# rohitgirdhar/AttentionalPoolingAction

Measured on AMD Instinct MI355X. Metric: images/sec attn-pool fwd+bwd, Nx14x14x2048, 393 classes, higher is better.
Workload: dtype f32; 1 GPU; cfg002 attentional-pooling head fwd + softmax-xent + bwd, per-GPU batch 32 x 14x14x2048 f32 features, K=393, M=1 (class-agnostic bottom-up map), dropout keep=0.2; X/dX rotated over 4 buffer sets (411 MB live); global_batch=32, parallelism=dp1, softmax_att=False, hip_graph=False, allreduce=none

## Files before the change

### attentionalpoolingaction_amd/csrc/apa_capi.hip

```cpp
#include <stdarg.h>
#include <stdio.h>

#include "../../include/apa_pose_cache.h"
#include "apa_internal.h"
#include "../../include/apa_clip_epoch.h"

namespace apa {

static thread_local char g_err[512] = "no error";

void set_error(const char* fmt, ...) {
  va_list ap;
  va_start(ap, fmt);
  vsnprintf(g_err, sizeof(g_err), fmt, ap);
  va_end(ap);
}

int hip_fail(hipError_t e, const char* what) {
  set_error("HIP error %d (%s) at %s", (int)e, hipGetErrorString(e), what);
  return APA_ERR_HIP;
}

__global__ void zero_words_kernel(uint32_t* __restrict__ p, size_t n) {
  const size_t stride = (size_t)gridDim.x * blockDim.x;
// ... 396 lines not shown
  if (d.ws_bytes < need) {
    set_error("%s: workspace too small (%zu < %zu = apa_attn_pool_rank_workspace_bytes)", fn, d.ws_bytes, need);
    return APA_ERR_WORKSPACE;
  }
  return APA_OK;
}

extern "C" size_t apa_attn_pool_rank_workspace_bytes(int N, int P, int C, int Ca, int K, int extra) {
  if (N <= 0 || P <= 0 || C <= 0 || Ca <= 0 || K <= 0 || extra < 1 || extra > APA_RANK_MAX - 1) return 0;
  return m1r_workspace_bytes(N, P, C, Ca, K, extra + 1);
}

static int rank_fwd_run(const PoolCall& d, const RankCall& rk, const M1Fwd& f) {
  M1Call c;
  const int rc = m1_call_fill(c, d, &f, nullptr);
  return rc != APA_OK ? rc : m1r_forward(c, rk, f);
}
static int rank_bwd_run(const PoolCall& d, const RankCall& rk, const M1Bwd& b) {
  M1Call c;
  const int rc = m1_call_fill(c, d, nullptr, &b);
  return rc != APA_OK ? rc : m1r_backward(c, rk, b);
}

extern "C" int apa_attn_pool_rank_fwd(const apa_rank_maps* rank, const void* X, const void* Xatt, const float* Wa,
                                      const float* ba, const float* Wt, const float* bt, float* logits, float* att,
                                      float* zsave, float* abar, void* ws, size_t ws_bytes, int N, int P, int C, int Ca,
                                      int K, int M, unsigned flags, float keep_prob, uint64_t seed, uint64_t offset,
                                      int dtype, void* stream) {
  const PoolCall d = pool_call({N, P, C, Ca, K, M, dtype}, flags, keep_prob, seed, offset, ws, ws_bytes, stream);
  const M1Fwd f{X, Xatt, Wa, ba, Wt, bt, logits, att, zsave, abar};
  RankCall rk = {};
  const int rc = rank_check("apa_attn_pool_rank_fwd", rank, d, &f, nullptr, &rk);
  return rc != APA_OK ? rc : rank_fwd_run(d, rk, f);
}

// ... 1143 lines not shown
```

### attentionalpoolingaction_amd/csrc/apa_internal.h

```cpp
#pragma once
#include <hip/hip_runtime.h>
#include <hip/hip_ext.h>
#include <stddef.h>
#include <stdint.h>
#include <stdlib.h>
#include <type_traits>

#include "../../include/apa.h"
#include "apa_colsum.h"
#include "apa_gather.h"

namespace apa {

void set_error(const char* fmt, ...);
int hip_fail(hipError_t e, const char* what);
int zero_fill(void* p, size_t bytes, hipStream_t st);

constexpr int APA_MAX_DEVICES = 64;
inline int current_device_slot() {
  int d = 0;
  if (hipGetDevice(&d) != hipSuccess || d < 0) d = 0;
  return d % APA_MAX_DEVICES;
}
template <typename T> struct PerDevice {
// ... 130 lines not shown
bool gemm_bf16_eligible(const GemmDesc& d);
int gemm_bf16_launch(const GemmDesc& d, int splits, int k_per_split, hipStream_t st);
bool gemm_bf16_twin_ok(const GemmDesc& d, int splits, int k_per_split);
bool gemm_bf16_zp_serves(const GemmDesc& d);
bool gemm_bf16_wide_serves(int M, int N, int K);
int gemm_bf16_wide_tile_rows(int M, int N, int K);
int gemm_bf16_mid_dropout(const void* A, long lda, const void* B, long ldb, void* C, long ldc, int M, int N,
                          int K, float inv_keep, const uint8_t* maskbits, hipStream_t st);

constexpr unsigned APA_PUBLIC_FLAGS = 0x3FFu;
constexpr unsigned APA_IFLAG_ATT_READY = 1u << 24;
constexpr unsigned APA_IFLAG_NO_ATT_WGRAD = 1u << 25;
constexpr unsigned APA_IFLAG_NO_DX = 1u << 26;
constexpr unsigned APA_IFLAG_FINALIZE_LAUNCH = 1u << 27;
constexpr unsigned APA_IFLAG_FOLD_TILE16 = 1u << 28;

struct M1Xent {
  const int64_t* labels = nullptr;
  float* loss = nullptr;
  float* G = nullptr;
  float gscale = 0.f, lscale = 0.f;
  bool done = false;
  bool deferred = false;
  float* logits = nullptr;
  float* probs = nullptr;
  int64_t* pred = nullptr;
  int kind = 0;
  const float* mlabels = nullptr;
  float pos_weight = 1.f;
  bool finished = false;
// ... 41 lines not shown
  int pool_bwd, bwd_w, bwd_pix;
  int fused, keep_bits, relu_input;
  int S, ppb, nblk, cw;
  int logits, logits_nv4, logits_nsub;
  int head, head_ug, head_mv;
  int gemv, reduce, rng_bump, cat_fwd, cat_bwd;
};
extern thread_local M1Trace* g_m1_trace;
inline M1Trace* m1_trace() { return g_m1_trace; }
struct M1FwdRoute {
  int folded;
  int launches;
};
extern thread_local unsigned g_m1_iflags;
extern thread_local M1FwdRoute g_m1_fwd_route;

enum M1Act { M1_ACT_ID = 0, M1_ACT_RELU = 1, M1_ACT_SOFTMAX = 2 };
struct M1Fwd {
  const void *X, *Xatt; const float *Wa, *ba, *Wt, *bt; float *logits, *att, *zsave, *abar; void* topdown = nullptr;
};
struct M1Bwd {
  const void *X, *Xatt; const float *Wa, *Wt, *bt, *att, *zsave, *abar, *G; void *dX, *dXatt; float *dWa, *dba, *dWt, *dbt;
};
struct M1Call {
  int N, P, C, Ca, K, dtype; unsigned flags; hipStream_t st; const CatFeat* cat;
  int act, pool_act;
  bool fused, train, rank1, ext, relu_input, no_dx, small, gemv2;
  M1Pool pool; M1Plan pl;
  float *pacc, *pstat, *pdwa, *pdba, *dz, *dzatt, *gemm_ws, *cat_e;
  float* sn;
  uint8_t* maskbits;
  const uint8_t* maskbits_in;
  RngKeyArgs key; float inv_keep; uint64_t* bump;
  const float* ex; float exs;
  hipEvent_t ev0, ev1, td_ready, grad_ready;
  bool gather; int T; M1Gather ga;
};
inline int64_t* m1_gathered_labels(void* ws, const M1Plan& pl) {
  return reinterpret_cast<int64_t*>(static_cast<char*>(ws) + pl.off_pdwa);
}
int m1_call_fill(M1Call& c, const PoolCall& d, const M1Fwd* f, const M1Bwd* b, const M1Xent* xf = nullptr);
int m1_forward(const M1Call& c, const M1Fwd& io, M1Xent* xf = nullptr);
int m1_backward(const M1Call& c, const M1Bwd& io, const M1Xent* xf = nullptr);
bool m1_supported(int C, int Ca, int dtype, bool fused);
bool m1_no_dx_supported(int C, int dtype, bool train);
template <typename F> inline int m1_fused_train(bool fused, bool train, F&& go) {
  if (fused) return train ? go(std::true_type{}, std::true_type{}) : go(std::true_type{}, std::false_type{});
  return train ? go(std::false_type{}, std::true_type{}) : go(std::false_type{}, std::false_type{});
}
template <typename Fn> inline int m1_pool_form(const M1Call& c, Fn&& go) {
  if (c.gather) return m1_fused_train(c.fused, c.train, [&](auto F, auto TR) { return go(F, TR, std::true_type{}); });
  return m1_fused_train(c.fused, c.train, [&](auto F, auto TR) { return go(F, TR, std::false_type{}); });
// ... 35 lines not shown
int m1r_forward(const M1Call& c, const RankCall& rk, const M1Fwd& io);
int m1r_backward(const M1Call& c, const RankCall& rk, const M1Bwd& io);
bool m1_cat_supported(int J);
int m1_cat_forward(const M1Call& c, const M1Fwd& io);
int m1_cat_backward(const M1Call& c, const M1Bwd& io);

bool m1_small_supported(int C, int K);
inline bool m1_small_route_ok(int C, int K, const float* G, const float* Wt, const float* zsave, bool any_ck = false) {
  return (any_ck || m1_small_supported(C, K)) && (((uintptr_t)G | (uintptr_t)Wt | (uintptr_t)zsave) & 15) == 0;
}
int m1_bwd_small(const float* G, const float* Wt, const float* zsave, const float* abar,
                 const float* bt, float* dz, float* dWt, float* dbt, float* sn, int N, int C, int K,
                 hipStream_t st);
bool m1_logits2_supported(int C, int K);
size_t m1_logits2_ws_bytes(int N, int C, int K);
struct M1Fold { const float* pacc; const float* pstat; int S, P; };
bool m1_logits2_fold_supported(int N, int C, int S);
int m1_logits2(float* z, const float* Wt, float* abar, const float* bt, float* logits,
               float* part_ws, int N, int C, int K, hipStream_t st, const M1Fold* fold = nullptr);
int m1_logits2_partials(float* z, const float* Wt, float* part_ws, int N, int C, int K, hipStream_t st,
                        const M1Fold* fold, int* nparts);
bool m1_logits_ml_supported(int N, int C, int K);
int m1_logits2_ml(float* z, const float* Wt, float* abar, const float* bt, const M1Xent& xf, float* logits,
                  float* part_ws, int N, int C, int K, hipStream_t st, const M1Fold* fold);
int ml_loss_rows(int kind, const float* labels, float pos_weight, const float* logits, float* loss, float* G, int N,
                 int K, float wt, float grad_scale, hipStream_t st);
int clip_loss_finish(const float* x, const float* dws, float* loss, float* dw, float* db, int B, int rows, int K,
                     float lscale, hipStream_t st);
int clip_scores_launch(const char* fn, int kind, const float* logits, const float* w, const float* b,
                       const int64_t* labels, float* pooled, float* tatt, float* scores, int64_t* pred, float* loss,
                       int B, int F, int K, hipStream_t st);
bool m1_bwd_head_supported(int N, int C, int K);
// ... 157 lines not shown
```

### attentionalpoolingaction_amd/csrc/apa_m1.hip

```cpp
#include <math.h>

#include "apa_device.h"
#include "apa_internal.h"

namespace apa {

__global__ __launch_bounds__(256) void m1_finalize_fwd_kernel(
    const float* __restrict__ pacc, const float* __restrict__ pstat, int P, int S, int C, int online_softmax, int cw,
    float* __restrict__ z, float* __restrict__ abar, float* __restrict__ att) {
  __shared__ float s_w[256];
  __shared__ float s_red[8];
  const int n = blockIdx.x;
  const int lane = threadIdx.x & 63, wave = threadIdx.x >> 6;
  const float invP = 1.0f / (float)P;
  const float* st = pstat + (size_t)n * S * 4;
  constexpr int FB = 16;
  const bool chan = (int)threadIdx.x < cw;
  const int v = chan ? blockIdx.y * cw + threadIdx.x : 0;
  const float* pa = pacc + (size_t)n * S * C + (v * 4 < C ? v * 4 : 0);
  float4 first[FB];
  if (chan) {
#pragma unroll
    for (int u = 0; u < FB; ++u)
      first[u] = *reinterpret_cast<const float4*>(pa + (size_t)min(u, S - 1) * C);
  }
  float m_s = -INFINITY, l_s = 0.f, a_s = 0.f;
  if ((int)threadIdx.x < S) {
    m_s = st[threadIdx.x * 4];
    l_s = st[threadIdx.x * 4 + 1];
    a_s = st[threadIdx.x * 4 + 2];
  }
  float M = 0.f, invL = 1.f, asum = 0.f;
  if (online_softmax) {
    float mw = wave_max(m_s);
    if (lane == 0) s_red[wave] = mw;
    __syncthreads();
    M = fmaxf(fmaxf(s_red[0], s_red[1]), fmaxf(s_red[2], s_red[3]));
    const float e = ((int)threadIdx.x < S) ? expf(m_s - M) : 0.f;
    float lw = wave_sum(l_s * e);
// ... 1 lines not shown
    __syncthreads();
    invL = 1.0f / ((s_red[4] + s_red[5]) + (s_red[6] + s_red[7]));
    s_w[threadIdx.x] = e * invL * invP;
  } else {
    float aw = wave_sum(a_s);
    if (lane == 0) s_red[wave] = aw;
    s_w[threadIdx.x] = invP;
    __syncthreads();
    asum = (s_red[0] + s_red[1]) + (s_red[2] + s_red[3]);
  }
  __syncthreads();
  if (chan && v * 4 < C) {
    float4 r = make_float4(0.f, 0.f, 0.f, 0.f);
#pragma unroll
    for (int u = 0; u < FB; ++u) {
      if (u < S) {
        const float w = s_w[u];
        r.x = fmaf(first[u].x, w, r.x); r.y = fmaf(first[u].y, w, r.y);
        r.z = fmaf(first[u].z, w, r.z); r.w = fmaf(first[u].w, w, r.w);
      }
    }
    for (int s0 = FB; s0 < S; s0 += FB) {
      float4 a[FB];
#pragma unroll
      for (int u = 0; u < FB; ++u)
        a[u] = *reinterpret_cast<const float4*>(pa + (size_t)min(s0 + u, S - 1) * C);
#pragma unroll
      for (int u = 0; u < FB; ++u) {
        const float w = s0 + u < S ? s_w[s0 + u] : 0.f;
        r.x = fmaf(a[u].x, w, r.x); r.y = fmaf(a[u].y, w, r.y);
        r.z = fmaf(a[u].z, w, r.z); r.w = fmaf(a[u].w, w, r.w);
      }
    }
    *reinterpret_cast<float4*>(z + (size_t)n * C + v * 4) = r;
  }
  if (blockIdx.y == 0) {
    if (online_softmax) {
      float tot = 0.f;
      for (int p = threadIdx.x; p < P; p += 256) {
        const float a = expf(att[(size_t)n * P + p] - M) * invL;
        att[(size_t)n * P + p] = a;
        tot += a;
      }
      tot = wave_sum(tot);
// ... 156 lines not shown
        dwa[e] = fmaf(g[u], x[e], dwa[e]);
      }
      if (STORE && active && p0 + u < p_end) st16(dXa + (size_t)(p0 + u) * Ca + v * EPV, Vec<T>::pack(o));
    }
  }
  if (active) {
#pragma unroll
    for (int e = 0; e < EPV; ++e) pdwa[(size_t)blockIdx.x * Ca + v * EPV + e] = dwa[e];
  }
  if (threadIdx.x == 0) pdba[blockIdx.x] = dba;
}

thread_local M1Trace* g_m1_trace = nullptr;
thread_local unsigned g_m1_iflags = 0;
thread_local M1FwdRoute g_m1_fwd_route = {0, 0};

bool m1_supported(int C, int Ca, int dtype, bool fused) {
  if (dtype == APA_DTYPE_FP8_E4M3) return fused && m1f_supported(C);
  const int epv = dtype == APA_DTYPE_BF16 ? 8 : 4;
  if (!fused && (Ca % epv != 0)) return false;
  return m1s_supported(C, dtype) || m1v_supported(C, dtype) || m1g_supported(C, dtype);
}

M1Plan m1_plan(int N, int P, int C, int Ca, int K) {
  M1Plan pl;
  int S = (512 + N / 2) / N;
  if (S < 1) S = 1;
  int maxS = P >= 8 ? P / 4 : 1;
  if (maxS > 256) maxS = 256;
  if (S > maxS) S = maxS;
// ... 40 lines not shown
  c.train = (flags & APA_FLAG_TRAIN) && keep_prob < 1.0f;
  c.act = (flags & APA_FLAG_SOFTMAX_ATT) ? M1_ACT_SOFTMAX
          : (flags & APA_FLAG_RELU_ATT) ? M1_ACT_RELU : M1_ACT_ID;
  c.pool_act = c.fused ? c.act : M1_ACT_ID;
  c.rank1 = b && (flags & APA_FLAG_DXATT_RANK1) != 0 && !c.fused;
  c.ext = c.train && rng_external(flags);
  c.relu_input = (flags & APA_FLAG_RELU_INPUT) != 0;
  c.no_dx = b && (flags & (APA_IFLAG_NO_DX | APA_FLAG_FROZEN_INPUT)) != 0;
  c.small = b && m1_small_route_ok(C, K, b->G, b->Wt, b->zsave);
  const int epv = dtype == APA_DTYPE_F32 ? 4 : 8;
  c.gemv2 = Ca % epv == 0 && Ca / epv <= 256;
  c.pool = dtype == APA_DTYPE_FP8_E4M3 ? M1_POOL_FP8
           : !c.ext && m1s_supported(C, dtype) ? M1_POOL_STREAM
           : !c.ext && m1v_supported(C, dtype) ? M1_POOL_VEC : M1_POOL_GENERIC;
  c.pl = m1_plan(N, P, C, Ca, K);
  char* w = static_cast<char*>(ws);
  c.pacc = reinterpret_cast<float*>(w + c.pl.off_pacc);
  c.pstat = reinterpret_cast<float*>(w + c.pl.off_pstat);
  c.pdwa = reinterpret_cast<float*>(w + c.pl.off_pdwa);
  c.pdba = reinterpret_cast<float*>(w + c.pl.off_pdba);
  c.sn = c.small ? c.pdba + c.pl.nblk : nullptr;
  c.dz = reinterpret_cast<float*>(w + c.pl.off_dz);
  c.dzatt = c.rank1 ? static_cast<float*>(b->dXatt) : reinterpret_cast<float*>(w + c.pl.off_dzatt);
  c.gemm_ws = reinterpret_cast<float*>(w + c.pl.off_gemm);
  c.cat_e = reinterpret_cast<float*>(w + c.pl.off_cat_e);
  c.maskbits = reinterpret_cast<uint8_t*>(w + c.pl.off_maskbits);
  c.maskbits_in = b && (flags & APA_FLAG_WS_FROM_FWD) ? c.maskbits : nullptr;
  c.key = rng_resolve(flags, keep_prob, seed, offset);
  c.inv_keep = c.train ? 1.0f / keep_prob : 1.0f;
  c.bump = (b && c.train && (flags & APA_FLAG_RNG_DEVICE)) ? reinterpret_cast<uint64_t*>(static_cast<uintptr_t>(offset))
// ... 2 lines not shown
  c.exs = cat ? 1.0f : 0.0f;
  c.ev0 = b ? hk.bwd0 : hk.fwd0; c.ev1 = b ? hk.bwd1 : hk.fwd1;
  c.gather = d.fc != nullptr;
  c.T = c.gather ? d.fc->cache_images : N;
  c.ga = M1Gather{nullptr, 0, nullptr, nullptr, nullptr};
  if (c.gather) {
    c.ga.index = d.fc->index; c.ga.T = c.T;
    if (f) {
      c.ga.status = d.fc->status;
      if (d.fc_labels) { c.ga.labels = d.fc_labels; c.ga.labels_out = m1_gathered_labels(ws, c.pl); }
    }
  }
  c.td_ready = hk.td_ready; c.grad_ready = hk.grad_ready;
  if (M1Trace* tr = m1_trace()) {
    tr->S = c.pl.S; tr->ppb = c.pl.ppb; tr->nblk = c.pl.nblk; tr->fused = c.fused; tr->relu_input = c.relu_input;
  }

  const bool cache_form = c.fused && c.act != M1_ACT_SOFTMAX && !c.relu_input && !c.ext && !cat && !(b && !c.no_dx) &&
                          !(flags & APA_IFLAG_NO_DX);
  if (c.pool == M1_POOL_FP8 && !(cache_form && m1f_supported(C))) {
    set_error("attn_pool M=1: APA_DTYPE_FP8_E4M3 serves the fused identity / relu head on frozen features only");
    return APA_ERR_UNSUPPORTED;
  }
  const bool pose_form = d.fc_pose && !c.fused && c.pool != M1_POOL_FP8 && c.act != M1_ACT_SOFTMAX && !c.relu_input &&
                         !c.ext && !cat && !(b && !c.no_dx) && !(flags & APA_IFLAG_NO_DX);
  if (c.gather && !cache_form && !pose_form) {
    set_error("attn_pool M=1: a feature cache serves the fused identity / relu head on frozen features only");
    return APA_ERR_UNSUPPORTED;
  }
  if (c.pool == M1_POOL_STREAM && !m1_pix_range_ok(P, c.pl.S)) {
// ... 63 lines not shown
  switch (c.pool) {
    case M1_POOL_STREAM: rc = m1s_launch_pool_fwd(c, io); break;
    case M1_POOL_VEC: rc = m1v_launch_pool_fwd(c, io); break;
    case M1_POOL_FP8: rc = m1f_launch_pool_fwd(c, io); break;
    default: rc = m1g_launch_pool_fwd(c, io);
  }
  if (rc != APA_OK) return rc;
  const int online = (c.fused && c.act == M1_ACT_SOFTMAX) ? 1 : 0;
  const bool xeval = xf && xf->probs;
  if (c.cat) xf = nullptr;
  const bool ml = xf && xf->kind != 0;
  const bool xroute = xf && (ml ? m1_logits_ml_supported(N, C, K) : m1_logits_xent_supported(N, C, K, xeval)) &&
                      m1_small_route_ok(C, K, xf->G, io.Wt, io.zsave, xeval);
  const bool l2route = m1_logits2_supported(C, K) && (reinterpret_cast<uintptr_t>(io.zsave) & 15) == 0;
  const bool fold = (xroute || l2route) && !((c.flags | g_m1_iflags) & APA_IFLAG_FINALIZE_LAUNCH) &&
                    c.act != M1_ACT_SOFTMAX && !c.cat && m1_logits2_fold_supported(N, C, c.pl.S) &&
                    ((reinterpret_cast<uintptr_t>(io.zsave) | reinterpret_cast<uintptr_t>(c.pacc)) & 15) == 0;
  const M1Fold mf{c.pacc, c.pstat, c.pl.S, c.P};
  int cw = 256;
  while (cw > 64 && (long)N * ((C + 4 * cw - 1) / (4 * cw)) < 256) cw >>= 1;
  if (tr) {
    tr->cw = cw;
    g_m1_fwd_route.folded = fold;
    g_m1_fwd_route.launches = (fold ? 0 : 1) + 2;
  }
  if (!fold) {
    hipLaunchKernelGGL(m1_finalize_fwd_kernel, dim3(N, (C + 4 * cw - 1) / (4 * cw)), dim3(256), 0, c.st, c.pacc,
                       c.pstat, c.P, c.pl.S, C, online, cw, io.zsave, io.abar, io.att);
    APA_LAUNCH_CHECK("m1_finalize_fwd_kernel");
  }
  if (c.td_ready) APA_HIP_CHECK(hipStreamWaitEvent(c.st, c.td_ready, 0));
  if (xroute) {
    if (ml) {
      if (tr) tr->logits = M1_LOGITS_ML;
      rc = m1_logits2_ml(io.zsave, io.Wt, io.abar, io.bt, *xf, io.logits, c.gemm_ws, N, C, K, c.st, fold ? &mf : nullptr);
      xf->finished = !m1_bwd_head_supported(N, C, K);
      if (rc == APA_OK && xf->finished)
        rc = clip_loss_finish(nullptr, nullptr, xf->loss, nullptr, nullptr, N, N, K, xf->lscale, c.st);
      xf->done = rc == APA_OK;
      return rc;
    }
    if (tr) tr->logits = xeval ? M1_LOGITS_XENT_PROBS : M1_LOGITS_XENT;
    rc = m1_logits2_xent(io.zsave, io.Wt, io.abar, io.bt, xf->labels, io.logits, xf->loss, xf->G, xf->gscale,
// ... 111 lines not shown
```

### attentionalpoolingaction_amd/csrc/apa_m1_probe.hip

```cpp
#include "apa_internal.h"

namespace {
constexpr int64_t M1_PROBE_VERSION = 1;

struct TraceScope {
  explicit TraceScope(apa::M1Trace* t) {
    if (t) *t = apa::M1Trace{};
    apa::g_m1_trace = t;
  }
  ~TraceScope() { apa::g_m1_trace = nullptr; }
};
}

extern "C" {

int64_t apa_probe_m1_version(void) { return M1_PROBE_VERSION; }
int64_t apa_probe_m1_trace_size(void) { return (int64_t)sizeof(apa::M1Trace); }

void apa_probe_m1_plan(int N, int P, int C, int Ca, int K, int64_t* out) {
  const apa::M1Plan pl = apa::m1_plan(N, P, C, Ca, K);
  out[0] = pl.S; out[1] = pl.ppb; out[2] = pl.nblk; out[3] = pl.lsplits;
}

int apa_probe_m1_support(int N, int C, int K, int dtype) {
// ... 18 lines not shown
  apa::M1Bwd b{};
  b.X = base; b.Xatt = xatt_is_x ? base : base + 16;
  b.Wt = reinterpret_cast<const float*>(base); b.zsave = b.Wt; b.G = b.Wt; b.att = b.Wt;
  b.dXatt = base;
  apa::PoolCall d{{N, P, C, Ca, K, 1, dtype}};
  d.flags = flags; d.keep_prob = keep_prob; d.seed = 1; d.offset = 2; d.ws = base;
  const apa::M1Fwd f{b.X, b.Xatt};
  apa::M1Xent xf;
  xf.done = loss_done != 0;
  const int rc = apa::m1_call_fill(c, d, bwd ? nullptr : &f, bwd ? &b : nullptr, &xf);
  out[0] = c.pl.S; out[1] = c.pl.ppb; out[2] = c.pl.nblk; out[3] = c.pl.lsplits; out[4] = (int64_t)c.pl.total;
  out[5] = c.pool; out[6] = c.small; out[7] = c.train; out[8] = c.fused; out[9] = (int64_t)c.pl.off_pacc;
  return rc;
}

int apa_probe_m1_fwd_ex(apa::M1Trace* t, const apa_hooks* hooks, const void* X, const void* Xatt, const float* Wa,
                        const float* ba, const float* Wt, const float* bt, float* logits, float* att, float* zsave,
                        float* abar, void* topdown, void* ws, size_t ws_bytes, int N, int P, int C, int Ca, int K,
                        int M, unsigned flags, float keep_prob, uint64_t seed, uint64_t offset, int dtype,
                        void* stream) {
  TraceScope s(t);
  return apa_attn_pool_fwd_ex(hooks, X, Xatt, Wa, ba, Wt, bt, logits, att, zsave, abar, topdown, ws, ws_bytes, N, P,
                              C, Ca, K, M, flags, keep_prob, seed, offset, dtype, stream);
}

int apa_probe_m1_bwd_ex(apa::M1Trace* t, const apa_hooks* hooks, const void* X, const void* Xatt, const float* Wa,
                        const float* ba, const float* Wt, const float* bt, const float* att, const float* zsave,
                        const float* abar, const float* G, void* dX, void* dXatt, float* dWa, float* dba,
                        float* dWt, float* dbt, void* ws, size_t ws_bytes, int N, int P, int C, int Ca, int K,
                        int M, unsigned flags, float keep_prob, uint64_t seed, uint64_t offset, int dtype,
// ... 87 lines not shown
```

### attentionalpoolingaction_amd/csrc/apa_m1_small.hip

```cpp
#include "apa_device.h"
#include "apa_internal.h"

namespace apa {

__device__ __forceinline__ f32x4 mfma16(float a, float b, f32x4 c) {
  return __builtin_amdgcn_mfma_f32_16x16x4f32(a, b, c, 0, 0, 0);
}

__global__ __launch_bounds__(256) void m1_logits_reduce_kernel(const float* __restrict__ part,
                                                               const float* __restrict__ pstat,
                                                               const float* __restrict__ bt, int N, int K,
                                                               int nchunks, int S, int P, float* abar,
                                                               float* __restrict__ logits) {
  const int idx = blockIdx.x * 256 + threadIdx.x;
  if (idx >= N * K) return;
  const int n = idx / K, k = idx - n * K;
  float ab = 0.f;
  if (pstat) ab = m1_abar_thread(pstat, n, S, P);
  const size_t stride = (size_t)N * K;
  float v[32];
  float acc = 0.f;
  for (int c = 0; c < nchunks; c += 32) {
#pragma unroll
    for (int u = 0; u < 32; ++u) v[u] = part[(size_t)min(c + u, nchunks - 1) * stride + idx];
// ... 332 lines not shown
  __syncthreads();
  const int row = tid >> 4, colr = tid & 15;
  float* out = part + (size_t)cx * N * K;
#pragma unroll
  for (int ni = 0; ni < 2; ++ni) {
#pragma unroll
    for (int j = 0; j < KG; ++j) {
      const int t = (ni * KG + j) * 256 + tid;
      const float sm = (red[t] + red[2 * KG * 256 + t]) + (red[4 * KG * 256 + t] + red[6 * KG * 256 + t]);
      const int n = n0 + ni * 16 + row, kt = gx * KG + j, k = kt * 16 + colr;
      if (n < N && kt < ktiles && k < K) out[(size_t)n * K + k] = sm;
    }
  }
}

template <int KG, int ROWS>
__global__ __launch_bounds__(256) void m1_logits2_fold_kernel(const float* __restrict__ pacc,
                                                              const float* __restrict__ Wt,
                                                              float* __restrict__ zsave,
                                                              float* __restrict__ part, int N, int C, int K,
                                                              int S, int P) {
  static_assert(ROWS == 8 || ROWS == 16, "half or full MFMA tiles");
  constexpr int RT = ROWS * 16;
  extern __shared__ __attribute__((aligned(16))) float red[];
  const int tid = threadIdx.x, wave = tid >> 6, lane = tid & 63;
  const int r = lane & 15, kq = lane >> 4;
  const int cx = blockIdx.x, gx = blockIdx.y, n0 = blockIdx.z * ROWS;
  const int ktiles = (K + 15) >> 4;
  const int n = min(n0 + (r & (ROWS - 1)), N - 1);
  const int cw = cx * 64 + wave * 16;
  const float invP = 1.0f / (float)P;
  int colj[KG];
#pragma unroll
  for (int j = 0; j < KG; ++j)
    colj[j] = min(min(gx * KG + j, ktiles - 1) * 16 + r, K - 1);
  constexpr int FB = 16;
  const float* pa = pacc + (size_t)n * S * C + cw + 4 * kq;
  float4 first[FB];
#pragma unroll
  for (int u = 0; u < FB; ++u) first[u] = *reinterpret_cast<const float4*>(pa + (size_t)min(u, S - 1) * C);
  __builtin_amdgcn_sched_barrier(0);
  float bw[KG][4];
#pragma unroll
  for (int j = 0; j < KG; ++j)
#pragma unroll
    for (int e = 0; e < 4; ++e) bw[j][e] = Wt[(size_t)(cw + 4 * kq + e) * K + colj[j]];
  __builtin_amdgcn_sched_barrier(0);
  float4 z = make_float4(0.f, 0.f, 0.f, 0.f);
#pragma unroll
  for (int u = 0; u < FB; ++u) {
    if (u < S) {
      z.x = fmaf(first[u].x, invP, z.x); z.y = fmaf(first[u].y, invP, z.y);
      z.z = fmaf(first[u].z, invP, z.z); z.w = fmaf(first[u].w, invP, z.w);
    }
  }
  if (gx == 0 && r < ROWS && n0 + r < N) *reinterpret_cast<float4*>(zsave + (size_t)(n0 + r) * C + cw + 4 * kq) = z;
  f32x4 acc[KG];
#pragma unroll
  for (int j = 0; j < KG; ++j) acc[j] = f32x4{0.f, 0.f, 0.f, 0.f};
  const float av[4] = {z.x, z.y, z.z, z.w};
#pragma unroll
  for (int e = 0; e < 4; ++e) {
#pragma unroll
    for (int j = 0; j < KG; ++j) acc[j] = mfma16(av[e], bw[j][e], acc[j]);
  }
  if (kq < ROWS / 4) {
// ... 368 lines not shown

static int logits2_nsub(int N, int C) { return (N >= 128 && C % 256 == 0) ? 4 : 1; }

static int launch_logits2(const float* z, const float* Wt, float* part_ws, int N, int C, int K, hipStream_t st) {
  constexpr int KG = 7;
  const int ktiles = (K + 15) / 16;
  const int nsub = logits2_nsub(N, C);
  if (M1Trace* t = m1_trace()) t->logits_nsub = nsub;
  dim3 grid(C / (64 * nsub), (ktiles + KG - 1) / KG, (N + 31) / 32);
  const size_t shm = (size_t)4 * 2 * KG * 256 * sizeof(float);
  hipLaunchKernelGGL((m1_logits2_kernel<KG>), grid, dim3(256), shm, st, z, Wt, part_ws, N, C, K, nsub);
  APA_LAUNCH_CHECK("m1_logits2_kernel");
  return APA_OK;
}

bool m1_logits2_fold_supported(int N, int C, int S) {
  return C % 64 == 0 && S >= 1 && S <= 16 && N >= 1 && N < 128;
}

static int launch_logits2_fold(const M1Fold& f, const float* Wt, float* zsave, float* part_ws, int N, int C, int K,
                               hipStream_t st) {
  const int ktiles = (K + 15) / 16, half = (ktiles + 1) / 2;
  const int kg = half <= 1 ? 1 : (half <= 2 ? 2 : (half <= 4 ? 4 : (half <= 7 ? 7 : 13)));
  if (M1Trace* t = m1_trace()) t->logits_nsub = 1;
  const int blocks8 = (C / 64) * ((ktiles + kg - 1) / kg) * ((N + 7) / 8);
  const int blocks16 = (C / 64) * ((ktiles + 6) / 7) * ((N + 15) / 16);
  const bool tile16 = (g_m1_iflags & APA_IFLAG_FOLD_TILE16) || (N > 8 && (blocks16 >= blocks8 || blocks16 >= 256));
  if (tile16) {
    dim3 grid(C / 64, (ktiles + 6) / 7, (N + 15) / 16);
    const size_t shm = (size_t)4 * 7 * 256 * sizeof(float);
    hipLaunchKernelGGL((m1_logits2_fold_kernel<7, 16>), grid, dim3(256), shm, st, f.pacc, Wt, zsave, part_ws, N, C, K,
                       f.S, f.P);
    APA_LAUNCH_CHECK("m1_logits2_fold_kernel");
    return APA_OK;
  }
  dim3 grid(C / 64, (ktiles + kg - 1) / kg, (N + 7) / 8);
  const size_t shm = (size_t)4 * kg * 128 * sizeof(float);
#define APA_LF(KG)                                                                                             \
  hipLaunchKernelGGL((m1_logits2_fold_kernel<KG, 8>), grid, dim3(256), shm, st, f.pacc, Wt, zsave, part_ws, N, \
                     C, K, f.S, f.P)
  if (kg == 1) APA_LF(1);
  else if (kg == 2) APA_LF(2);
  else if (kg == 4) APA_LF(4);
  else if (kg == 7) APA_LF(7);
  else APA_LF(13);
#undef APA_LF
  APA_LAUNCH_CHECK("m1_logits2_fold_kernel");
  return APA_OK;
}

int m1_logits2(float* z, const float* Wt, float* abar, const float* bt, float* logits,
               float* part_ws, int N, int C, int K, hipStream_t st, const M1Fold* fold) {
  const int rc = fold ? launch_logits2_fold(*fold, Wt, z, part_ws, N, C, K, st)
                      : launch_logits2(z, Wt, part_ws, N, C, K, st);
  if (rc != APA_OK) return rc;
// ... 135 lines not shown
```

### attentionalpoolingaction_amd/csrc/apa_m1_stream.hip

```cpp
#include <math.h>

#include "apa_device.h"
#include "apa_internal.h"

#ifndef APA_BWD_NT_LOAD
#define APA_BWD_NT_LOAD false
#endif

namespace apa {

namespace {
template <int PIX>
__device__ __forceinline__ float block_dots(const float (&d)[PIX], float* sm, int wave, int lane) {
  const int l16 = lane & 15;
  float mine = 0.f;
#pragma unroll
  for (int i = 0; i < PIX; ++i) {
    const float r = row_sum16(d[i]);
    mine = (l16 == i) ? r : mine;
  }
  sm[wave * 64 + l16 * 4 + (lane >> 4)] = mine;
  __syncthreads();
  const float4 v = *reinterpret_cast<const float4*>(&sm[lane * 4]);
  float s = (v.x + v.y) + (v.z + v.w);
// ... 47 lines not shown
    const int p = min(q0 + i, p_last);
#pragma unroll
    for (int j = 0; j < VW; ++j) {
      const T* src = xim + (size_t)p * C + cbase + j * 64 * EPV;
#if APA_M1S_OPAQUE_X
      const u4 v = NT ? __builtin_nontemporal_load((gvec_ptr)src) : *(gvec_ptr)src;
      xr[i][j] = make_uint4(v.x, v.y, v.z, v.w);
#else
      xr[i][j] = NT ? ld16_nt(src) : ld16(src);
#endif
    }
  }
  __builtin_amdgcn_sched_barrier(0);
}

struct ChunkRange { int q0, np; };
template <int PIX>
__device__ __forceinline__ ChunkRange chunk_range(int p_begin, int p_end, int ch) {
  ChunkRange r;
  r.q0 = p_begin + ch * PIX;
  r.np = min(PIX, p_end - r.q0);
  return r;
}

template <typename T, int VW, int PIX, bool FUSED, bool TRAIN>
struct FwdState {
  static constexpr int EPV = Vec<T>::EPV;
  static constexpr int EPL = VW * EPV;
  float wa[FUSED ? EPL : 1];
  float acc[EPL];
// ... 87 lines not shown
      if (BPL == 1) {
        const uint32_t b1 = (uint32_t)__builtin_amdgcn_mov_dpp((int)lbits, 0x39, 0xf, 0xf, true);
        const uint32_t b2 = (uint32_t)__builtin_amdgcn_mov_dpp((int)lbits, 0x4E, 0xf, 0xf, true);
        const uint32_t b3 = (uint32_t)__builtin_amdgcn_mov_dpp((int)lbits, 0x93, 0xf, 0xf, true);
        const uint32_t w = (lbits & 0xffu) | ((b1 & 0xffu) << 8) | ((b2 & 0xffu) << 16) | (b3 << 24);
        if ((lane & 3) == 0) *reinterpret_cast<uint32_t*>(dst) = w;
      } else {
        const uint32_t b1 = (uint32_t)__builtin_amdgcn_mov_dpp((int)lbits, 0xB1, 0xf, 0xf, true);
        const uint32_t w = (lbits & 0xffffu) | (b1 << 16);
        if ((lane & 1) == 0) *reinterpret_cast<uint32_t*>(dst) = w;
      }
    }
  }
}

template <typename T, int VW, int PIX, bool FUSED, bool TRAIN, bool SM, bool RIN = false, bool GATHER = false>
__global__ __launch_bounds__(256, 2) void m1s_pool_fwd_kernel(
    const T* __restrict__ X, int P, int S, int nblk, int act, const float* __restrict__ Wa,
    const float* __restrict__ ba, float* __restrict__ att, float* __restrict__ pacc,
    float* __restrict__ pstat, float inv_keep, uint32_t thresh, uint64_t seed, uint64_t offset,
    const uint64_t* __restrict__ offset_dev, uint8_t* __restrict__ maskbits, M1GatherArg<GATHER> g) {
  constexpr int EPV = Vec<T>::EPV;
  constexpr int EPL = VW * EPV;
  constexpr int CW = EPL * 64;
  constexpr int C = CW * 4;
  __shared__ __attribute__((aligned(16))) float sm_x[APA_M1S_NB][256];

  const unsigned blk = (unsigned)xcd_remap(blockIdx.x, nblk);
  const int n = (int)(blk / (unsigned)S), s = (int)(blk % (unsigned)S);
  const int wave = threadIdx.x >> 6, lane = threadIdx.x & 63;
  int p_begin, p_end;
  m1_pix_range(s, P, S, p_begin, p_end);
  const int npt = p_end - p_begin;
  const int nchunk = (npt + PIX - 1) / PIX;
  const int cbase = wave * CW + lane * EPV;

  const T* xim = opaque_global(X + (size_t)(GATHER ? m1_src_image(n, g) : n) * P * C);
  float* att_im = att + (size_t)n * P;
  uint8_t* bits_im = TRAIN ? maskbits + (size_t)n * P * MaskBytes<EPL>::BPP : nullptr;

  const int p_last = p_end - 1;
  constexpr int NB = APA_M1S_NB;
  uint4 xr[NB][PIX][VW];
  const int l16 = lane & 15;
  const float* att_rd = opaque_global(static_cast<const float*>(att_im));
// ... 27 lines not shown

  for (int ch = 0; ch < nchunk; ch += NB) {
#pragma unroll
    for (int u = 0; u < NB; ++u) {
      if (u > 0 && ch + u >= nchunk) break;
      constexpr int NBm1 = NB - 1;
      const int slot = (u + NBm1) % NB;
      if (!FUSED) av_r[slot] = att_rd[min(p_begin + (ch + u + NBm1) * PIX + l16, p_last)];
      load_chunk<T, VW, PIX>(xr[slot], xim, p_begin + (ch + u + NBm1) * PIX, p_last, C, cbase);
      fwd_chunk<T, VW, PIX, FUSED, TRAIN, SM, RIN>(st, xr[u], chunk_range<PIX>(p_begin, p_end, ch + u), sm_x[u], att_im,
                                                   n, P, C, cbase, wave, lane, act, inv_keep, thresh, k0, k1, bits_im,
                                                   av_r[u]);
    }
  }

  float* pa = pacc + (size_t)blk * C + cbase;
#pragma unroll
  for (int j = 0; j < VW; ++j) {
#pragma unroll
    for (int e = 0; e < EPV; e += 4) {
      const int i = j * EPV + e;
      *reinterpret_cast<float4*>(pa + j * 64 * EPV + e) =
          make_float4(st.acc[i], st.acc[i + 1], st.acc[i + 2], st.acc[i + 3]);
    }
  }
  m1_gather_note(n, s == 0 && threadIdx.x == 0, g);
  if (threadIdx.x == 0) {
    pstat[blk * 4 + 0] = (FUSED && SM) ? st.m_run : 0.f;
    pstat[blk * 4 + 1] = st.l_run;
    pstat[blk * 4 + 2] = st.a_sum;
    pstat[blk * 4 + 3] = 0.f;
  }
}

template <typename T, int VW, int PIX, bool FUSED, bool TRAIN>
struct BwdState {
  static constexpr int EPV = Vec<T>::EPV;
  static constexpr int EPL = VW * EPV;
  float dzr[EPL];
  float wa[FUSED ? EPL : 1];
  float dwa[FUSED ? EPL : 1];
  float dba_acc, sn, corr;
// ... 234 lines not shown
  const int epv = dtype == APA_DTYPE_BF16 ? 8 : 4;
  if (C % (256 * epv) != 0) return false;
  const int vw = C / (256 * epv);
  if (dtype == APA_DTYPE_BF16) return vw == 1;
  return vw == 1 || vw == 2 || vw == 4;
}

template <typename T, int VW> constexpr int kPix = sizeof(T) == 2 ? 2 : (VW == 4 ? 2 : 1);

template <typename T, int VW>
static int launch_fwd_t(const M1Call& c, const M1Fwd& io) {
  constexpr int PIX = kPix<T, VW>;
  if (M1Trace* t = m1_trace()) { t->pool_fwd = M1_POOL_STREAM; t->fwd_w = VW; t->fwd_pix = PIX; }
  m1_pool_form(c, [&](auto F, auto TR, auto G) {
    constexpr bool f = decltype(F)::value, t = decltype(TR)::value, g = decltype(G)::value;
    auto arm = [&](auto SM) {
      constexpr bool sm = decltype(SM)::value;
      auto k = m1s_pool_fwd_kernel<T, VW, PIX, f, t, sm, false, g>;
      if constexpr (f && !g) {
        if (c.relu_input) k = m1s_pool_fwd_kernel<T, VW, PIX, true, t, sm, true>;
      }
      return k;
    };
    auto kernel = arm(std::false_type{});
    if constexpr (f && !g) {
      if (c.pool_act == M1_ACT_SOFTMAX) kernel = arm(std::true_type{});
    }
    launch_ev(kernel, dim3(c.pl.nblk), dim3(256), 0, c.st, c.ev0, c.ev1, static_cast<const T*>(io.X), c.P, c.pl.S,
              c.pl.nblk, c.pool_act, io.Wa, io.ba, io.att, c.pacc, c.pstat, c.inv_keep, c.key.thresh, c.key.seed,
              c.key.offset, c.key.offset_dev, c.maskbits, m1_gather_arg<g>(c));
    return APA_OK;
  });
  APA_LAUNCH_CHECK("m1s_pool_fwd_kernel");
  return APA_OK;
}

template <typename T, int VW>
static int launch_bwd_t(const M1Call& c, const M1Bwd& io) {
  constexpr int PIX = kPix<T, VW>;
  M1Trace* const tr = m1_trace();
  if (tr) { tr->pool_bwd = M1_POOL_STREAM; tr->bwd_w = VW; tr->bwd_pix = PIX; }
  const uint8_t* mbits = c.relu_input ? nullptr : c.maskbits_in;
  bool bits = false;
// ... 56 lines not shown
```

Before: 731,800 images/sec.

## Pair adjacent pool blocks into 512-thread blocks and merge partials in LDS

The f32 streaming pool forward now launches half as many blocks. Each block has 512 threads and handles two adjacent pixel slices, and the two accumulators are merged through shared memory before one row is written. This halves the pacc rows that the finalize or fold-logits kernels must read and reduce, and a smaller fold instance (FB=8) is added for the reduced row count. The cost is an extra LDS buffer, block-wide barriers that match the partner's chunk count, and lower occupancy (launch bounds 512,1).

```diff
diff --git a/attentionalpoolingaction_amd/csrc/apa_capi.hip b/attentionalpoolingaction_amd/csrc/apa_capi.hip
--- a/attentionalpoolingaction_amd/csrc/apa_capi.hip
+++ b/attentionalpoolingaction_amd/csrc/apa_capi.hip
@@ -434,11 +434,13 @@
 static int rank_fwd_run(const PoolCall& d, const RankCall& rk, const M1Fwd& f) {
   M1Call c;
   const int rc = m1_call_fill(c, d, &f, nullptr);
+  m1_call_full_rows(c, false);
   return rc != APA_OK ? rc : m1r_forward(c, rk, f);
 }
 static int rank_bwd_run(const PoolCall& d, const RankCall& rk, const M1Bwd& b) {
   M1Call c;
   const int rc = m1_call_fill(c, d, nullptr, &b);
+  m1_call_full_rows(c, true);
   return rc != APA_OK ? rc : m1r_backward(c, rk, b);
 }
 
diff --git a/attentionalpoolingaction_amd/csrc/apa_internal.h b/attentionalpoolingaction_amd/csrc/apa_internal.h
--- a/attentionalpoolingaction_amd/csrc/apa_internal.h
+++ b/attentionalpoolingaction_amd/csrc/apa_internal.h
@@ -168,6 +168,7 @@
 constexpr unsigned APA_IFLAG_NO_DX = 1u << 26;
 constexpr unsigned APA_IFLAG_FINALIZE_LAUNCH = 1u << 27;
 constexpr unsigned APA_IFLAG_FOLD_TILE16 = 1u << 28;
+constexpr unsigned APA_IFLAG_UNPAIRED = 1u << 29;
 
 struct M1Xent {
   const int64_t* labels = nullptr;
@@ -239,6 +240,8 @@
 };
 extern thread_local unsigned g_m1_iflags;
 extern thread_local M1FwdRoute g_m1_fwd_route;
+struct M1Rows { int fwd, bwd; };
+extern thread_local M1Rows g_m1_rows;
 
 enum M1Act { M1_ACT_ID = 0, M1_ACT_RELU = 1, M1_ACT_SOFTMAX = 2 };
 struct M1Fwd {
@@ -252,6 +255,8 @@
   int act, pool_act;
   bool fused, train, rank1, ext, relu_input, no_dx, small, gemv2;
   M1Pool pool; M1Plan pl;
+  int nrows;
+  bool paired() const { return nrows != pl.nblk; }
   float *pacc, *pstat, *pdwa, *pdba, *dz, *dzatt, *gemm_ws, *cat_e;
   float* sn;
   uint8_t* maskbits;
@@ -261,6 +266,10 @@
   hipEvent_t ev0, ev1, td_ready, grad_ready;
   bool gather; int T; M1Gather ga;
 };
+inline void m1_call_full_rows(M1Call& c, bool bwd) {
+  c.nrows = c.pl.nblk;
+  if (m1_trace()) (bwd ? g_m1_rows.bwd : g_m1_rows.fwd) = c.nrows;
+}
 inline int64_t* m1_gathered_labels(void* ws, const M1Plan& pl) {
   return reinterpret_cast<int64_t*>(static_cast<char*>(ws) + pl.off_pdwa);
 }
@@ -326,8 +335,8 @@
                  hipStream_t st);
 bool m1_logits2_supported(int C, int K);
 size_t m1_logits2_ws_bytes(int N, int C, int K);
-struct M1Fold { const float* pacc; const float* pstat; int S, P; };
-bool m1_logits2_fold_supported(int N, int C, int S);
+struct M1Fold { const float* pacc; const float* pstat; int S, P, rows; };
+bool m1_logits2_fold_supported(int N, int C, int rows);
 int m1_logits2(float* z, const float* Wt, float* abar, const float* bt, float* logits,
                float* part_ws, int N, int C, int K, hipStream_t st, const M1Fold* fold = nullptr);
 int m1_logits2_partials(float* z, const float* Wt, float* part_ws, int N, int C, int K, hipStream_t st,
diff --git a/attentionalpoolingaction_amd/csrc/apa_m1.hip b/attentionalpoolingaction_amd/csrc/apa_m1.hip
--- a/attentionalpoolingaction_amd/csrc/apa_m1.hip
+++ b/attentionalpoolingaction_amd/csrc/apa_m1.hip
@@ -6,8 +6,8 @@
 namespace apa {
 
 __global__ __launch_bounds__(256) void m1_finalize_fwd_kernel(
-    const float* __restrict__ pacc, const float* __restrict__ pstat, int P, int S, int C, int online_softmax, int cw,
-    float* __restrict__ z, float* __restrict__ abar, float* __restrict__ att) {
+    const float* __restrict__ pacc, const float* __restrict__ pstat, int P, int S, int R, int C, int online_softmax,
+    int cw, float* __restrict__ z, float* __restrict__ abar, float* __restrict__ att) {
   __shared__ float s_w[256];
   __shared__ float s_red[8];
   const int n = blockIdx.x;
@@ -17,12 +17,12 @@
   constexpr int FB = 16;
   const bool chan = (int)threadIdx.x < cw;
   const int v = chan ? blockIdx.y * cw + threadIdx.x : 0;
-  const float* pa = pacc + (size_t)n * S * C + (v * 4 < C ? v * 4 : 0);
+  const float* pa = pacc + (size_t)n * R * C + (v * 4 < C ? v * 4 : 0);
   float4 first[FB];
   if (chan) {
 #pragma unroll
     for (int u = 0; u < FB; ++u)
-      first[u] = *reinterpret_cast<const float4*>(pa + (size_t)min(u, S - 1) * C);
+      first[u] = *reinterpret_cast<const float4*>(pa + (size_t)min(u, R - 1) * C);
   }
   float m_s = -INFINITY, l_s = 0.f, a_s = 0.f;
   if ((int)threadIdx.x < S) {
@@ -54,20 +54,20 @@
     float4 r = make_float4(0.f, 0.f, 0.f, 0.f);
 #pragma unroll
     for (int u = 0; u < FB; ++u) {
-      if (u < S) {
+      if (u < R) {
         const float w = s_w[u];
         r.x = fmaf(first[u].x, w, r.x); r.y = fmaf(first[u].y, w, r.y);
         r.z = fmaf(first[u].z, w, r.z); r.w = fmaf(first[u].w, w, r.w);
       }
     }
-    for (int s0 = FB; s0 < S; s0 += FB) {
+    for (int s0 = FB; s0 < R; s0 += FB) {
       float4 a[FB];
 #pragma unroll
       for (int u = 0; u < FB; ++u)
-        a[u] = *reinterpret_cast<const float4*>(pa + (size_t)min(s0 + u, S - 1) * C);
+        a[u] = *reinterpret_cast<const float4*>(pa + (size_t)min(s0 + u, R - 1) * C);
 #pragma unroll
       for (int u = 0; u < FB; ++u) {
-        const float w = s0 + u < S ? s_w[s0 + u] : 0.f;
+        const float w = s0 + u < R ? s_w[s0 + u] : 0.f;
         r.x = fmaf(a[u].x, w, r.x); r.y = fmaf(a[u].y, w, r.y);
         r.z = fmaf(a[u].z, w, r.z); r.w = fmaf(a[u].w, w, r.w);
       }
@@ -254,6 +254,7 @@
 thread_local M1Trace* g_m1_trace = nullptr;
 thread_local unsigned g_m1_iflags = 0;
 thread_local M1FwdRoute g_m1_fwd_route = {0, 0};
+thread_local M1Rows g_m1_rows = {0, 0};
 
 bool m1_supported(int C, int Ca, int dtype, bool fused) {
   if (dtype == APA_DTYPE_FP8_E4M3) return fused && m1f_supported(C);
@@ -324,6 +325,9 @@
            : !c.ext && m1s_supported(C, dtype) ? M1_POOL_STREAM
            : !c.ext && m1v_supported(C, dtype) ? M1_POOL_VEC : M1_POOL_GENERIC;
   c.pl = m1_plan(N, P, C, Ca, K);
+  const bool paired = f && c.pool == M1_POOL_STREAM && dtype == APA_DTYPE_F32 && c.pl.S % 2 == 0 &&
+                      c.pool_act != M1_ACT_SOFTMAX && !(g_m1_iflags & APA_IFLAG_UNPAIRED);
+  c.nrows = paired ? c.pl.nblk / 2 : c.pl.nblk;
   char* w = static_cast<char*>(ws);
   c.pacc = reinterpret_cast<float*>(w + c.pl.off_pacc);
   c.pstat = reinterpret_cast<float*>(w + c.pl.off_pstat);
@@ -356,6 +360,7 @@
   c.td_ready = hk.td_ready; c.grad_ready = hk.grad_ready;
   if (M1Trace* tr = m1_trace()) {
     tr->S = c.pl.S; tr->ppb = c.pl.ppb; tr->nblk = c.pl.nblk; tr->fused = c.fused; tr->relu_input = c.relu_input;
+    (b ? g_m1_rows.bwd : g_m1_rows.fwd) = c.nrows;
   }
 
   const bool cache_form = c.fused && c.act != M1_ACT_SOFTMAX && !c.relu_input && !c.ext && !cat && !(b && !c.no_dx) &&
@@ -449,9 +454,10 @@
                       m1_small_route_ok(C, K, xf->G, io.Wt, io.zsave, xeval);
   const bool l2route = m1_logits2_supported(C, K) && (reinterpret_cast<uintptr_t>(io.zsave) & 15) == 0;
   const bool fold = (xroute || l2route) && !((c.flags | g_m1_iflags) & APA_IFLAG_FINALIZE_LAUNCH) &&
-                    c.act != M1_ACT_SOFTMAX && !c.cat && m1_logits2_fold_supported(N, C, c.pl.S) &&
+                    c.act != M1_ACT_SOFTMAX && !c.cat && m1_logits2_fold_supported(N, C, c.nrows / N) &&
+                    c.pl.S <= 16 &&
                     ((reinterpret_cast<uintptr_t>(io.zsave) | reinterpret_cast<uintptr_t>(c.pacc)) & 15) == 0;
-  const M1Fold mf{c.pacc, c.pstat, c.pl.S, c.P};
+  const M1Fold mf{c.pacc, c.pstat, c.pl.S, c.P, c.nrows / N};
   int cw = 256;
   while (cw > 64 && (long)N * ((C + 4 * cw - 1) / (4 * cw)) < 256) cw >>= 1;
   if (tr) {
@@ -461,7 +467,7 @@
   }
   if (!fold) {
     hipLaunchKernelGGL(m1_finalize_fwd_kernel, dim3(N, (C + 4 * cw - 1) / (4 * cw)), dim3(256), 0, c.st, c.pacc,
-                       c.pstat, c.P, c.pl.S, C, online, cw, io.zsave, io.abar, io.att);
+                       c.pstat, c.P, c.pl.S, c.nrows / N, C, online, cw, io.zsave, io.abar, io.att);
     APA_LAUNCH_CHECK("m1_finalize_fwd_kernel");
   }
   if (c.td_ready) APA_HIP_CHECK(hipStreamWaitEvent(c.st, c.td_ready, 0));
diff --git a/attentionalpoolingaction_amd/csrc/apa_m1_probe.hip b/attentionalpoolingaction_amd/csrc/apa_m1_probe.hip
--- a/attentionalpoolingaction_amd/csrc/apa_m1_probe.hip
+++ b/attentionalpoolingaction_amd/csrc/apa_m1_probe.hip
@@ -56,6 +56,57 @@
   return rc;
 }
 
+void apa_probe_m1_rows(int64_t* out) { out[0] = apa::g_m1_rows.fwd; out[1] = apa::g_m1_rows.bwd; }
+
+int apa_probe_m1_call_rows(int bwd, int xatt_is_x, int unpaired, int N, int P, int C, int Ca, int K, unsigned flags,
+                           float keep_prob, int dtype, int64_t* out) {
+  alignas(16) static char base[64];
+  apa::M1Call c;
+  apa::M1Bwd b{};
+  b.X = base; b.Xatt = xatt_is_x ? base : base + 16;
+  b.Wt = reinterpret_cast<const float*>(base); b.zsave = b.Wt; b.G = b.Wt; b.att = b.Wt;
+  b.dXatt = base;
+  apa::PoolCall d{{N, P, C, Ca, K, 1, dtype}};
+  d.flags = flags; d.keep_prob = keep_prob; d.seed = 1; d.offset = 2; d.ws = base;
+  const apa::M1Fwd f{b.X, b.Xatt};
+  const unsigned saved = apa::g_m1_iflags;
+  if (unpaired == 1) apa::g_m1_iflags |= apa::APA_IFLAG_UNPAIRED;
+  const int rc = apa::m1_call_fill(c, d, bwd ? nullptr : &f, bwd ? &b : nullptr, nullptr);
+  if (unpaired == 2) apa::m1_call_full_rows(c, bwd != 0);
+  apa::g_m1_iflags = saved;
+  out[0] = c.nrows; out[1] = c.pl.nblk; out[2] = c.pl.S; out[3] = (int64_t)c.pl.total;
+  return rc;
+}
+
+namespace {
+struct UnpairedScope {
+  unsigned saved;
+  UnpairedScope() : saved(apa::g_m1_iflags) { apa::g_m1_iflags |= apa::APA_IFLAG_UNPAIRED; }
+  ~UnpairedScope() { apa::g_m1_iflags = saved; }
+};
+}
+int apa_probe_m1_fwd_unpaired(apa::M1Trace* t, const apa_hooks* hooks, const void* X, const void* Xatt, const float* Wa,
+                              const float* ba, const float* Wt, const float* bt, float* logits, float* att,
+                              float* zsave, float* abar, void* topdown, void* ws, size_t ws_bytes, int N, int P, int C,
+                              int Ca, int K, int M, unsigned flags, float keep_prob, uint64_t seed, uint64_t offset,
+                              int dtype, void* stream) {
+  TraceScope s(t);
+  UnpairedScope u;
+  return apa_attn_pool_fwd_ex(hooks, X, Xatt, Wa, ba, Wt, bt, logits, att, zsave, abar, topdown, ws, ws_bytes, N, P,
+                              C, Ca, K, M, flags, keep_prob, seed, offset, dtype, stream);
+}
+int apa_probe_m1_bwd_unpaired(apa::M1Trace* t, const apa_hooks* hooks, const void* X, const void* Xatt, const float* Wa,
+                              const float* ba, const float* Wt, const float* bt, const float* att, const float* zsave,
+                              const float* abar, const float* G, void* dX, void* dXatt, float* dWa, float* dba,
+                              float* dWt, float* dbt, void* ws, size_t ws_bytes, int N, int P, int C, int Ca, int K,
+                              int M, unsigned flags, float keep_prob, uint64_t seed, uint64_t offset, int dtype,
+                              void* stream) {
+  TraceScope s(t);
+  UnpairedScope u;
+  return apa_attn_pool_bwd_ex(hooks, X, Xatt, Wa, ba, Wt, bt, att, zsave, abar, G, dX, dXatt, dWa, dba, dWt, dbt,
+                              ws, ws_bytes, N, P, C, Ca, K, M, flags, keep_prob, seed, offset, dtype, stream);
+}
+
 int apa_probe_m1_fwd_ex(apa::M1Trace* t, const apa_hooks* hooks, const void* X, const void* Xatt, const float* Wa,
                         const float* ba, const float* Wt, const float* bt, float* logits, float* att, float* zsave,
                         float* abar, void* topdown, void* ws, size_t ws_bytes, int N, int P, int C, int Ca, int K,
diff --git a/attentionalpoolingaction_amd/csrc/apa_m1_small.hip b/attentionalpoolingaction_amd/csrc/apa_m1_small.hip
--- a/attentionalpoolingaction_amd/csrc/apa_m1_small.hip
+++ b/attentionalpoolingaction_amd/csrc/apa_m1_small.hip
@@ -370,12 +370,12 @@
   }
 }
 
-template <int KG, int ROWS>
+template <int KG, int ROWS, int FB = 16>
 __global__ __launch_bounds__(256) void m1_logits2_fold_kernel(const float* __restrict__ pacc,
                                                               const float* __restrict__ Wt,
                                                               float* __restrict__ zsave,
                                                               float* __restrict__ part, int N, int C, int K,
-                                                              int S, int P) {
+                                                              int R, int P) {
   static_assert(ROWS == 8 || ROWS == 16, "half or full MFMA tiles");
   constexpr int RT = ROWS * 16;
   extern __shared__ __attribute__((aligned(16))) float red[];
@@ -390,11 +390,10 @@
 #pragma unroll
   for (int j = 0; j < KG; ++j)
     colj[j] = min(min(gx * KG + j, ktiles - 1) * 16 + r, K - 1);
-  constexpr int FB = 16;
-  const float* pa = pacc + (size_t)n * S * C + cw + 4 * kq;
+  const float* pa = pacc + (size_t)n * R * C + cw + 4 * kq;
   float4 first[FB];
 #pragma unroll
-  for (int u = 0; u < FB; ++u) first[u] = *reinterpret_cast<const float4*>(pa + (size_t)min(u, S - 1) * C);
+  for (int u = 0; u < FB; ++u) first[u] = *reinterpret_cast<const float4*>(pa + (size_t)min(u, R - 1) * C);
   __builtin_amdgcn_sched_barrier(0);
   float bw[KG][4];
 #pragma unroll
@@ -405,7 +404,7 @@
   float4 z = make_float4(0.f, 0.f, 0.f, 0.f);
 #pragma unroll
   for (int u = 0; u < FB; ++u) {
-    if (u < S) {
+    if (u < R) {
       z.x = fmaf(first[u].x, invP, z.x); z.y = fmaf(first[u].y, invP, z.y);
       z.z = fmaf(first[u].z, invP, z.z); z.w = fmaf(first[u].w, invP, z.w);
     }
@@ -804,8 +803,8 @@
   return APA_OK;
 }
 
-bool m1_logits2_fold_supported(int N, int C, int S) {
-  return C % 64 == 0 && S >= 1 && S <= 16 && N >= 1 && N < 128;
+bool m1_logits2_fold_supported(int N, int C, int rows) {
+  return C % 64 == 0 && rows >= 1 && rows <= 16 && N >= 1 && N < 128;
 }
 
 static int launch_logits2_fold(const M1Fold& f, const float* Wt, float* zsave, float* part_ws, int N, int C, int K,
@@ -819,8 +818,12 @@
   if (tile16) {
     dim3 grid(C / 64, (ktiles + 6) / 7, (N + 15) / 16);
     const size_t shm = (size_t)4 * 7 * 256 * sizeof(float);
-    hipLaunchKernelGGL((m1_logits2_fold_kernel<7, 16>), grid, dim3(256), shm, st, f.pacc, Wt, zsave, part_ws, N, C, K,
-                       f.S, f.P);
+    if (f.rows <= 8)
+      hipLaunchKernelGGL((m1_logits2_fold_kernel<7, 16, 8>), grid, dim3(256), shm, st, f.pacc, Wt, zsave, part_ws, N, C,
+                         K, f.rows, f.P);
+    else
+      hipLaunchKernelGGL((m1_logits2_fold_kernel<7, 16>), grid, dim3(256), shm, st, f.pacc, Wt, zsave, part_ws, N, C, K,
+                         f.rows, f.P);
     APA_LAUNCH_CHECK("m1_logits2_fold_kernel");
     return APA_OK;
   }
@@ -828,7 +831,7 @@
   const size_t shm = (size_t)4 * kg * 128 * sizeof(float);
 #define APA_LF(KG)                                                                                             \
   hipLaunchKernelGGL((m1_logits2_fold_kernel<KG, 8>), grid, dim3(256), shm, st, f.pacc, Wt, zsave, part_ws, N, \
-                     C, K, f.S, f.P)
+                     C, K, f.rows, f.P)
   if (kg == 1) APA_LF(1);
   else if (kg == 2) APA_LF(2);
   else if (kg == 4) APA_LF(4);
diff --git a/attentionalpoolingaction_amd/csrc/apa_m1_stream.hip b/attentionalpoolingaction_amd/csrc/apa_m1_stream.hip
--- a/attentionalpoolingaction_amd/csrc/apa_m1_stream.hip
+++ b/attentionalpoolingaction_amd/csrc/apa_m1_stream.hip
@@ -85,6 +85,52 @@
   __builtin_amdgcn_sched_barrier(0);
 }
 
+struct PairId { int blk, quad, wave, tid; };
+template <bool PAIR>
+__device__ __forceinline__ PairId pair_id(int nblk) {
+  PairId r;
+  if (PAIR) {
+    r.quad = __builtin_amdgcn_readfirstlane((int)(threadIdx.x >> 8));
+    r.blk = 2 * xcd_remap(blockIdx.x, nblk >> 1) + r.quad;
+  } else {
+    r.quad = 0;
+    r.blk = xcd_remap(blockIdx.x, nblk);
+  }
+  r.tid = threadIdx.x & 255;
+  r.wave = r.tid >> 6;
+  return r;
+}
+template <int PIX>
+__device__ __forceinline__ int partner_chunks(int s, int P, int S) {
+  int b, e;
+  m1_pix_range(s ^ 1, P, S, b, e);
+  return (e - b + PIX - 1) / PIX;
+}
+template <int EPL, int EPV>
+__device__ __forceinline__ void pair_merge(float (&acc)[EPL], float* sm, int quad, int cbase) {
+#pragma unroll
+  for (int j = 0; j < EPL / EPV; ++j) {
+#pragma unroll
+    for (int e = 0; e < EPV; e += 4) {
+      const int i = j * EPV + e;
+      if (quad == 1)
+        *reinterpret_cast<float4*>(sm + cbase + j * 64 * EPV + e) = make_float4(acc[i], acc[i + 1], acc[i + 2], acc[i + 3]);
+    }
+  }
+  __syncthreads();
+  if (quad == 0) {
+#pragma unroll
+    for (int j = 0; j < EPL / EPV; ++j) {
+#pragma unroll
+      for (int e = 0; e < EPV; e += 4) {
+        const int i = j * EPV + e;
+        const float4 o = *reinterpret_cast<const float4*>(sm + cbase + j * 64 * EPV + e);
+        acc[i] = acc[i] + o.x; acc[i + 1] = acc[i + 1] + o.y; acc[i + 2] = acc[i + 2] + o.z; acc[i + 3] = acc[i + 3] + o.w;
+      }
+    }
+  }
+}
+
 struct ChunkRange { int q0, np; };
 template <int PIX>
 __device__ __forceinline__ ChunkRange chunk_range(int p_begin, int p_end, int ch) {
@@ -202,8 +248,9 @@
   }
 }
 
-template <typename T, int VW, int PIX, bool FUSED, bool TRAIN, bool SM, bool RIN = false, bool GATHER = false>
-__global__ __launch_bounds__(256, 2) void m1s_pool_fwd_kernel(
+template <typename T, int VW, int PIX, bool FUSED, bool TRAIN, bool SM, bool RIN = false, bool GATHER = false,
+          bool PAIR = false>
+__global__ __launch_bounds__(PAIR ? 512 : 256, PAIR ? 1 : 2) void m1s_pool_fwd_kernel(
     const T* __restrict__ X, int P, int S, int nblk, int act, const float* __restrict__ Wa,
     const float* __restrict__ ba, float* __restrict__ att, float* __restrict__ pacc,
     float* __restrict__ pstat, float inv_keep, uint32_t thresh, uint64_t seed, uint64_t offset,
@@ -212,11 +259,15 @@
   constexpr int EPL = VW * EPV;
   constexpr int CW = EPL * 64;
   constexpr int C = CW * 4;
-  __shared__ __attribute__((aligned(16))) float sm_x[APA_M1S_NB][256];
-
-  const unsigned blk = (unsigned)xcd_remap(blockIdx.x, nblk);
+  static_assert(!(PAIR && SM), "softmax instances keep one block per logical block");
+  __shared__ __attribute__((aligned(16))) float sm_xq[PAIR ? 2 : 1][APA_M1S_NB][256];
+  __shared__ __attribute__((aligned(16))) float sm_row[PAIR ? C : 4];
+
+  const PairId id = pair_id<PAIR>(nblk);
+  const unsigned blk = (unsigned)id.blk;
   const int n = (int)(blk / (unsigned)S), s = (int)(blk % (unsigned)S);
-  const int wave = threadIdx.x >> 6, lane = threadIdx.x & 63;
+  const int wave = id.wave, lane = threadIdx.x & 63;
+  float (*sm_x)[256] = sm_xq[id.quad];
   int p_begin, p_end;
   m1_pix_range(s, P, S, p_begin, p_end);
   const int npt = p_end - p_begin;
@@ -274,18 +325,25 @@
     }
   }
 
-  float* pa = pacc + (size_t)blk * C + cbase;
-#pragma unroll
-  for (int j = 0; j < VW; ++j) {
-#pragma unroll
-    for (int e = 0; e < EPV; e += 4) {
-      const int i = j * EPV + e;
-      *reinterpret_cast<float4*>(pa + j * 64 * EPV + e) =
-          make_float4(st.acc[i], st.acc[i + 1], st.acc[i + 2], st.acc[i + 3]);
-    }
-  }
-  m1_gather_note(n, s == 0 && threadIdx.x == 0, g);
-  if (threadIdx.x == 0) {
+  if constexpr (PAIR) {
+    if (FUSED)
+      for (int ch = nchunk, nc = partner_chunks<PIX>(s, P, S); ch < nc; ++ch) __syncthreads();
+    pair_merge<EPL, EPV>(st.acc, sm_row, id.quad, cbase);
+  }
+  if (!PAIR || id.quad == 0) {
+    float* pa = pacc + (size_t)(PAIR ? blk >> 1 : blk) * C + cbase;
+#pragma unroll
+    for (int j = 0; j < VW; ++j) {
+#pragma unroll
+      for (int e = 0; e < EPV; e += 4) {
+        const int i = j * EPV + e;
+        *reinterpret_cast<float4*>(pa + j * 64 * EPV + e) =
+            make_float4(st.acc[i], st.acc[i + 1], st.acc[i + 2], st.acc[i + 3]);
+      }
+    }
+  }
+  m1_gather_note(n, s == 0 && id.tid == 0, g);
+  if (id.tid == 0) {
     pstat[blk * 4 + 0] = (FUSED && SM) ? st.m_run : 0.f;
     pstat[blk * 4 + 1] = st.l_run;
     pstat[blk * 4 + 2] = st.a_sum;
@@ -550,19 +608,24 @@
   if (M1Trace* t = m1_trace()) { t->pool_fwd = M1_POOL_STREAM; t->fwd_w = VW; t->fwd_pix = PIX; }
   m1_pool_form(c, [&](auto F, auto TR, auto G) {
     constexpr bool f = decltype(F)::value, t = decltype(TR)::value, g = decltype(G)::value;
-    auto arm = [&](auto SM) {
-      constexpr bool sm = decltype(SM)::value;
-      auto k = m1s_pool_fwd_kernel<T, VW, PIX, f, t, sm, false, g>;
+    auto arm = [&](auto SM, auto PR) {
+      constexpr bool sm = decltype(SM)::value, pr = decltype(PR)::value;
+      auto k = m1s_pool_fwd_kernel<T, VW, PIX, f, t, sm, false, g, pr>;
       if constexpr (f && !g) {
-        if (c.relu_input) k = m1s_pool_fwd_kernel<T, VW, PIX, true, t, sm, true>;
+        if (c.relu_input) k = m1s_pool_fwd_kernel<T, VW, PIX, true, t, sm, true, false, pr>;
       }
       return k;
     };
-    auto kernel = arm(std::false_type{});
+    const std::true_type yes; const std::false_type no;
+    auto kernel = arm(no, no);
+    const bool pair = c.paired();
+    if constexpr (sizeof(T) == 4) {
+      if (pair) kernel = arm(no, yes);
+    }
     if constexpr (f && !g) {
-      if (c.pool_act == M1_ACT_SOFTMAX) kernel = arm(std::true_type{});
-    }
-    launch_ev(kernel, dim3(c.pl.nblk), dim3(256), 0, c.st, c.ev0, c.ev1, static_cast<const T*>(io.X), c.P, c.pl.S,
+      if (c.pool_act == M1_ACT_SOFTMAX) kernel = arm(yes, no);
+    }
+    launch_ev(kernel, dim3(c.nrows), dim3(pair ? 512 : 256), 0, c.st, c.ev0, c.ev1, static_cast<const T*>(io.X), c.P, c.pl.S,
               c.pl.nblk, c.pool_act, io.Wa, io.ba, io.att, c.pacc, c.pstat, c.inv_keep, c.key.thresh, c.key.seed,
               c.key.offset, c.key.offset_dev, c.maskbits, m1_gather_arg<g>(c));
     return APA_OK;
```

Result: faster. 749,400 images/sec, median of 6 (+2.4%).
